# joaotavora/raytracing-one-weekend

Measured on AMD Instinct MI355X. Metric: Msamples/sec (W×H×spp) on cover scene; achieved HBM GB/s vs peak, higher is better.
Workload: dtype f64

## Files before the change

raytracing-one-weekend_amd/csrc/rtow_trace_body.h:

```cpp

#include <hip/hip_runtime.h>
#include <stdint.h>
#include <type_traits>

#include "rtow_device.h"

#ifndef RTOW_SUFFIX
#error "define RTOW_SUFFIX"
#endif
#define RTOW_CAT2(a, b) a##b
#define RTOW_CAT(a, b) RTOW_CAT2(a, b)

namespace rtow {
namespace {
#include "rtow_trace_math.h"
#include "rtow_trace_rng.h"
#include "rtow_trace_hit.h"
#include "rtow_trace_stamps.h"
#include "rtow_trace_bvh.h"
#include "rtow_trace_grid.h"
#include "rtow_trace_bvh4.h"
#ifndef RTOW_FAST_MATH
#include "rtow_trace_reftree.h"
#endif
#include "rtow_kernel_frame.h"

__device__ __forceinline__ uint32_t fastdiv(uint32_t n, FastDiv f) {
  const uint32_t t = __umulhi(n, f.magic);
  return f.shift == 255u ? n : (((n - t) >> 1) + t) >> f.shift;
}

constexpr uint32_t kItemBatch = 64;

__device__ __forceinline__ uint32_t lane_read(uint32_t src, uint32_t v) {
  return (uint32_t)__builtin_amdgcn_ds_bpermute((int)(src << 2), (int)v);
}
__device__ __forceinline__ double lane_read(uint32_t src, double v) {
  const unsigned long long b = (unsigned long long)__double_as_longlong(v);
  const uint32_t lo = lane_read(src, (uint32_t)b), hi = lane_read(src, (uint32_t)(b >> 32));
  return __longlong_as_double((long long)(((unsigned long long)hi << 32) | lo));
}
__device__ __forceinline__ double wave_bcast_f64(double v, int src_lane) {
  const unsigned long long b = (unsigned long long)__double_as_longlong(v);
  const uint32_t lo = (uint32_t)__builtin_amdgcn_readlane((int)(uint32_t)b, src_lane);
  const uint32_t hi = (uint32_t)__builtin_amdgcn_readlane((int)(uint32_t)(b >> 32), src_lane);
  return __longlong_as_double((long long)(((unsigned long long)hi << 32) | lo));
}

struct ItemPool {
  uint32_t next = 0, end = 0;
  unsigned long long seen = 0ull;
};

__device__ __forceinline__ FetchHead load_fetch_head(const RTOW_CONST FetchHead *p) {
  FetchHead h;
  h.n_items = p->n_items, h.n_items_first = p->n_items_first, h.empty_batch = p->empty_batch, h.W = p->W;
  h.partials = p->partials, h.counters = p->counters;
  return h;
}
__device__ __forceinline__ FetchDecode load_fetch_decode(const RTOW_CONST FetchDecode *p) {
  FetchDecode d;
  d.tile_w_log2 = p->tile_w_log2, d.tile_h_log2 = p->tile_h_log2, d.tile_table = p->tile_table;
  d.div_ns = FastDiv{p->div_ns.magic, p->div_ns.shift}, d.div_tpr = FastDiv{p->div_tpr.magic, p->div_tpr.shift};
  d.div_tpr_n = p->div_tpr_n, d.nstreams = p->nstreams, d.div_tile = FastDiv{p->div_tile.magic, p->div_tile.shift};
  d.rank = p->rank, d.nranks = p->nranks, d.tile_rows = p->tile_rows;
  d.sample_base = p->sample_base, d.spt = p->spt, d.spt_last = p->spt_last, d.npix_local = p->npix_local;
  return d;
}

__device__ __forceinline__ unsigned long long take_items(ItemPool &pool, unsigned long long need_mask, unsigned lane,
                                                         uint32_t n_waves, const FetchHead &kp) {
  const uint32_t want = (uint32_t)__popcll(need_mask);
  const uint32_t avail = pool.end - pool.next;
  const uint32_t rank = (uint32_t)__popcll(need_mask & ((1ull << lane) - 1ull));
  unsigned long long mine = (unsigned long long)pool.next + rank;
  if (want > avail) {
    const unsigned long long left =
        (unsigned long long)kp.n_items > pool.seen ? (unsigned long long)kp.n_items - pool.seen : 0ull;
#ifdef RTOW_NO_SHRINK
    uint32_t batch = kItemBatch;
    (void)left;
#else
    const bool sky = pool.seen >= (unsigned long long)kp.n_items_first;
    const uint32_t batch_max = sky ? kp.empty_batch : kItemBatch;
    uint32_t batch = (uint32_t)((sky ? left * (unsigned long long)(batch_max >> 6) : left) / ((unsigned long long)n_waves * 4ull));
    batch = batch > batch_max ? batch_max : batch;
    batch = batch < want - avail ? want - avail : batch;
#endif
    const int leader = __ffsll((long long)need_mask) - 1;
    unsigned long long base = pool.seen;
    if (pool.seen < (unsigned long long)kp.n_items) {
      if ((int)lane == leader) base = atomicAdd(&kp.counters[0], (unsigned long long)batch);
      base = __shfl(base, leader);
    }
    pool.seen = base + batch;
    if (rank >= avail) mine = base + (rank - avail);
    const unsigned long long nn = base + (want - avail), ne = base + batch;
    const unsigned long long cap = (unsigned long long)kp.n_items;
    pool.next = (uint32_t)(nn < cap ? nn : cap);
    pool.end = (uint32_t)(ne < cap ? ne : cap);
  } else {
    pool.next += want;
  }
  return mine;
}

struct ItemPos {
  uint32_t item, j, gi, sample0;
  int32_t count;
};
__device__ __forceinline__ ItemPos decode_item(const RTOW_CONST TraceParams *kp, const FetchHead &fh, uint32_t mine) {
  ItemPos ip;
  const FetchDecode kd = load_fetch_decode(kp);
  const uint32_t npix_local = kd.npix_local;
  const uint32_t qi = fh.n_items - 1u - mine;
  if (kd.tile_h_log2 == 0u) {
    const uint32_t k = fastdiv(qi, FastDiv{kp->div_npix.magic, kp->div_npix.shift});
    const uint32_t lp = qi - k * npix_local;
    const uint32_t lr = fastdiv(lp, FastDiv{kp->div_w.magic, kp->div_w.shift});
    ip.j = lp - lr * (uint32_t)fh.W;
    ip.item = k * npix_local + lp;
    const uint32_t q = fastdiv(lr, FastDiv{kd.div_tile.magic, kd.div_tile.shift});
    const uint32_t rr = lr - q * (uint32_t)kd.tile_rows;
    ip.gi = (q * (uint32_t)kd.nranks + (uint32_t)kd.rank) * (uint32_t)kd.tile_rows + rr;
    ip.sample0 = kd.sample_base + k * (uint32_t)kd.spt;
    ip.count = k + 1u == (uint32_t)kd.nstreams ? kd.spt_last : kd.spt;
    return ip;
  }
  const uint32_t g64 = qi >> 6, w = qi & 63u;
  const RTOW_CONST uint32_t *table = (const RTOW_CONST uint32_t *)kd.tile_table;
  ip.item = ip.j = ip.gi = ip.sample0 = 0u;
  ip.count = 0;
  for (;;) {
    const uint32_t ug = (uint32_t)__builtin_amdgcn_readfirstlane((int)g64);
    const uint32_t t = fastdiv(ug, FastDiv{kd.div_ns.magic, kd.div_ns.shift});
    const uint32_t k = ug - t * (uint32_t)kd.nstreams;
    const uint32_t tile = table[t];
    const uint32_t tr = fastdiv(tile, FastDiv{kd.div_tpr.magic, kd.div_tpr.shift});
    const uint32_t tc = tile - tr * kd.div_tpr_n;
    const uint32_t lr0 = tr << kd.tile_h_log2;
    const uint32_t q = fastdiv(lr0, FastDiv{kd.div_tile.magic, kd.div_tile.shift});
    const uint32_t gi0 = (q * (uint32_t)kd.nranks + (uint32_t)kd.rank) * (uint32_t)kd.tile_rows + (lr0 - q * (uint32_t)kd.tile_rows);
    const uint32_t item0 = k * npix_local + (tile << 6);
    const uint32_t j0 = tc << kd.tile_w_log2;
    const uint32_t s0 = kd.sample_base + k * (uint32_t)kd.spt;
    const int32_t cnt = k + 1u == (uint32_t)kd.nstreams ? kd.spt_last : kd.spt;
    if (g64 == ug) {
      ip.item = item0 + w;
      ip.j = j0 + (w & ((1u << kd.tile_w_log2) - 1u));
      ip.gi = gi0 + (w >> kd.tile_w_log2);
      ip.sample0 = s0;
      ip.count = cnt;
      break;
    }
  }
  return ip;
}

__device__ __forceinline__ void camera_ray(const TraceParams &P, Rng &g, uint32_t k0, uint32_t k1, uint32_t j,
                                           uint32_t gi, V3 &ro, V3 &rd, real &rtime) {
  g.r = 0u;
  const int from_top_i = P.H - (int)gi - 1;
  uint32_t o0, o1, o2, o3;
  philox4x32(g.r, g.sample, g.pixel, 0u, k0, k1, o0, o1, o2, o3);
  g.r += 1u;
  real ju, jv, jt, px, py;
  jitter_from_block(o0, o1, o2, ju, jv, jt);
  lens_from_block(o0, o1, o2, o3, px, py);
  const real u = fast_div((real)(int)j + ju, (real)(P.W - 1));
  const real v = fast_div((real)from_top_i + jv, (real)(P.H - 1));
#ifdef RTOW_REAL_F32
  const RTOW_CONST float *cm = (const RTOW_CONST float *)P.cam32;
#else
  cdptr cm = (cdptr)(const double *)P.cam;
#endif
  const real lens = cm[18], ct0 = cm[19], ct1 = cm[20];
  const real rdx = lens * px, rdy = lens * py;
  const V3 offset = V3{cm[3], cm[4], cm[5]} * rdx + V3{cm[6], cm[7], cm[8]} * rdy;
  const V3 from = V3{cm[0], cm[1], cm[2]} + offset;
  rd = V3{cm[15], cm[16], cm[17]} + u * V3{cm[9], cm[10], cm[11]} + v * V3{cm[12], cm[13], cm[14]} - from;
  ro = from;
  rtime = jt * (ct1 - ct0) + ct0;
}

__device__ __forceinline__ bool scatter_dir(Rng &g, uint32_t k0, uint32_t k1, int kind, real m_fuzz, real m_ir, V3 rd,
                                            V3 normal, bool front, V3 &dir) {
  uint32_t o0, o1, o2, o3;
  philox4x32(g.r, g.sample, g.pixel, 0u, k0, k1, o0, o1, o2, o3);
  g.r += 1u;
  V3 dirbase = {0, 0, 0};
  if (kind == 2) {
    const real ir = m_ir;
    const V3 unit = normalize(rd);
    const real cos_theta = dot(-unit, normal);
    const real sin_theta = fast_sqrt(real(1.0) - cos_theta * cos_theta);
    const real ratio = front ? fast_rcp(ir) : ir;
    bool refl = ratio * sin_theta > real(1.0);
    if (!refl) {
      real r0 = fast_div(real(1.0) - ratio, real(1.0) + ratio);
      r0 = r0 * r0;
      const real x = real(1.0) - cos_theta;
      const real x2 = x * x;
      const real R = r0 + (real(1.0) - r0) * (x2 * x2 * x);
      refl = R > coin_from_block(o0, o1, o3);
    }
    dirbase = refl ? reflect(unit, normal) : refract(unit, normal, ratio);
  } else if (kind == 1) {
    dirbase = reflect(rd, normal);
  }
  const V3 rnd = ball_from_block(o0, o1, o2, o3);
  bool absorbed = false;
  if (kind == 0) {
    absorbed = rabs(normal.x - rnd.x) < real(1e-8) && rabs(normal.y - rnd.y) < real(1e-8) &&
               rabs(normal.z - rnd.z) < real(1e-8);
    dir = normal + rnd;
  } else {
    dir = dirbase + m_fuzz * rnd;
  }
  return !absorbed;
}

template <int KERNEL, bool LDS, bool STAMPS = false, int SPEC = 0, bool COUNT = true>
__global__ void __launch_bounds__(KERNEL >= 2 && KERNEL <= 4 ? 1024 : 256)
    RTOW_CAT(rtow_trace_, RTOW_SUFFIX)(const TraceParams P) {
  const DevScene &sc = P.sc;
  const uint32_t k0 = P.seed_lo, k1 = P.seed_hi;
  const unsigned lane = lane_id();
  [[maybe_unused]] const uint32_t lane_g = blockIdx.x * blockDim.x + threadIdx.x;

  Image<LDS> im;
  [[maybe_unused]] Bvh4Reader<LDS> im4;
  stage_scene<KERNEL, LDS>(sc, im, im4);

  bool done = false;
  bool need_sample = true;
  bool pending_hit = false;
  int s_left = 0;
  uint32_t item = 0xffffffffu;
  uint32_t j = 0;
  uint32_t gi = 0;
  V3d acc = {0.0, 0.0, 0.0};
  V3 ro = {0, 0, 0}, rd = {0, 0, 1};
  real rtime = 0;
  int depth = 0;
  [[maybe_unused]] int nb = 0;
#ifdef RTOW_FAST_MATH
  V3 throughput = {1, 1, 1};
#endif
  Rng g = {0, 0, 0};
#ifdef RTOW_TAILSTAT
  constexpr bool kCount = true;
#else
  constexpr bool kCount = COUNT || STAMPS;
#endif
  WalkCount<kCount> nseg, nnode, nprim;
  [[maybe_unused]] float t_resume = 0.0f;
  [[maybe_unused]] uint32_t w_cur = 0x1fffffu, w_sa = 0u;
  Closest best;
  best.t = 0;
  best.prim = -1;
  bool helping = false;
  bool holding = false;
  uint32_t partners = 0u;
  int n_out = 0;
  uint32_t tail_left = P.tail_bound;
  asm volatile("" : "+v"(tail_left));
  ItemPool pool;
  const uint32_t n_waves = (gridDim.x * blockDim.x) >> 6;
#ifdef RTOW_TAILSTAT
  unsigned long long ts_start = __builtin_amdgcn_s_memrealtime(), ts_empty = 0ull;
  uint32_t ts_trips = 0u, ts_trips_after = 0u, ts_live = 0u, ts_left = 0u, ts_pool = 0u;
#endif
  Stamps<STAMPS> stamps;
  stamps.start();
  unsigned long long t_empty = 0ull;
  unsigned long long trips_after_empty = 0ull;
  if constexpr (STAMPS) {
    if (lane == 0) atomicMin(P.t_origin, (unsigned long long)__builtin_amdgcn_s_memrealtime());
  }

  for (;;) {
    bool need_item = false;
    if (!done && need_sample && s_left <= 0) {
      if (helping) {
        helping = false;
        holding = true;
        done = true;
      } else if (n_out == 0) {
        need_item = true;
      }
    }
    unsigned long long need_mask = __ballot(need_item);
    if (need_mask != 0ull && (uint32_t)__popcll(need_mask) < P.fetch_votes && __ballot(!done && !need_item) != 0ull) {
      need_mask = 0ull;
      need_item = false;
    }
    if (need_mask != 0ull) {
      const RTOW_CONST TraceParams *kp = (const RTOW_CONST TraceParams *)__builtin_amdgcn_kernarg_segment_ptr();
      asm volatile("" : "+s"(kp));
      const FetchHead fh = load_fetch_head(kp);
      if (need_item && item != 0xffffffffu) {
        double *dst = fh.partials + (size_t)item * 3;
        dst[0] = acc.x;
        dst[1] = acc.y;
        dst[2] = acc.z;
        item = 0xffffffffu;
      }
      const unsigned long long mine = take_items(pool, need_mask, lane, n_waves, fh);
      if (need_item) {
        if (mine >= (unsigned long long)fh.n_items) {
          done = true;
#ifdef RTOW_TAILSTAT
          if (ts_empty == 0ull) ts_empty = 1ull;
#endif
          if constexpr (STAMPS) {
            if (t_empty == 0ull) t_empty = __builtin_amdgcn_s_memrealtime();
          }
        } else {
          const ItemPos ip = decode_item(kp, fh, (uint32_t)mine);
          item = ip.item;
          j = ip.j;
          gi = ip.gi;
          g.pixel = gi * (uint32_t)fh.W + j;
          g.sample = ip.sample0;
          s_left = ip.count;
          acc = {0.0, 0.0, 0.0};
        }
      }
    }
#ifdef RTOW_TAILSTAT
    {
      const bool first = __ballot(ts_empty == 1ull) != 0ull && __ballot(ts_empty > 1ull) == 0ull;
      if (first) {
        const unsigned long long now = __builtin_amdgcn_s_memrealtime();
        ts_live = (uint32_t)__popcll(__ballot(!done));
        uint32_t sl = (!done && s_left > 0) ? (uint32_t)s_left : 0u;
        for (int off = 32; off >= 1; off >>= 1) sl += __shfl_xor(sl, off);
        ts_left = sl;
        ts_pool = pool.end - pool.next;
        ts_empty = now < 2ull ? 2ull : now;
      } else if (__ballot(ts_empty > 1ull) != 0ull) {
        ts_empty = (unsigned long long)__shfl((long long)ts_empty, __ffsll((long long)__ballot(ts_empty > 1ull)) - 1);
      }
      ++ts_trips;
      if (__ballot(ts_empty > 1ull) != 0ull) ++ts_trips_after;
    }
#endif
    if (__ballot(done) != 0ull) {
#ifdef RTOW_DONATE_R2
      const bool ready = !done && need_sample && s_left <= 0 && n_out > 0;
      if (__ballot(ready) != 0ull) {
        const uint32_t h = partners & 63u;
        const uint32_t src = ready ? h : lane;
        const uint32_t partner_holds = lane_read(src, (uint32_t)holding);
        const bool take = ready && partner_holds != 0u;
        const V3d c = {lane_read(src, acc.x), lane_read(src, acc.y), lane_read(src, acc.z)};
        const uint32_t ow = holding ? partners : lane;
        const bool o_take = lane_read(ow, (uint32_t)take) != 0u;
        const uint32_t o_h = lane_read(ow, h);
        if (take) {
          acc = acc + c;
          partners >>= 6;
          --n_out;
        }
        if (holding && o_take && o_h == lane) holding = false;
      }
      const bool can_give = !done && !helping && s_left >= 2 && n_out < 5;
#else
      unsigned long long rm = __ballot(!done && need_sample && s_left <= 0 && n_out > 0);
      while (rm != 0ull) {
        const int o = __ffsll((long long)rm) - 1;
        rm &= rm - 1ull;
        const uint32_t want_sample = (uint32_t)__builtin_amdgcn_readlane((int)g.sample, o);
        const uint32_t want_pixel = (uint32_t)__builtin_amdgcn_readlane((int)g.pixel, o);
        const unsigned long long held =
            __ballot(holding && partners == (uint32_t)o && g.sample == want_sample + 1u && g.pixel == want_pixel);
        if (held != 0ull) {
          const int h = __ffsll((long long)held) - 1;
          const V3d c = {wave_bcast_f64(acc.x, h), wave_bcast_f64(acc.y, h), wave_bcast_f64(acc.z, h)};
          if ((int)lane == o) {
            acc = acc + c;
            ++g.sample;
            --n_out;
          }
          if ((int)lane == h) holding = false;
          if (__builtin_amdgcn_readlane(n_out, o) > 0) rm |= 1ull << o;
        }
      }
      const bool can_give = !done && !helping && s_left >= 2;
#endif
      const bool can_help = done && !holding;
      const unsigned long long gm = __ballot(can_give), hm = __ballot(can_help);
      if (gm != 0ull && hm != 0ull) {
        const uint32_t ng = (uint32_t)__popcll(gm), nh = (uint32_t)__popcll(hm);
        const uint32_t cnt = ng < nh ? ng : nh;
        const uint32_t grank = lanes_below(gm), hrank = lanes_below(hm);
        const uint32_t giver_k = (uint32_t)__builtin_amdgcn_ds_permute(
            (int)((can_give ? grank : ng + (lane - grank)) << 2), (int)lane);
        const bool gives = can_give && grank < cnt;
        const bool helps = can_help && hrank < cnt;
        const uint32_t my_giver = lane_read(helps ? hrank : lane, giver_k);
#ifdef RTOW_DONATE_R2
        const uint32_t helper_k = (uint32_t)__builtin_amdgcn_ds_permute(
            (int)((can_help ? hrank : nh + (lane - hrank)) << 2), (int)lane);
        const uint32_t my_helper = lane_read(gives ? grank : lane, helper_k);
#endif
        const uint32_t gsrc = helps ? my_giver : lane;
        const uint32_t o_j = lane_read(gsrc, j), o_gi = lane_read(gsrc, gi);
        const uint32_t o_pixel = lane_read(gsrc, g.pixel), o_sample = lane_read(gsrc, g.sample);
        const uint32_t o_left = lane_read(gsrc, (uint32_t)s_left);
        if (gives) {
          s_left -= 1;
#ifdef RTOW_DONATE_R2
          partners = (partners << 6) | my_helper;
#endif
          ++n_out;
        }
        if (helps) {
          j = o_j;
          gi = o_gi;
          g.pixel = o_pixel;
          g.sample = o_sample + o_left - 1u;
          s_left = 1;
          need_sample = true;
          acc = {0.0, 0.0, 0.0};
          helping = true;
          done = false;
          partners = my_giver;
        }
      }
      if (tail_left == 0u) {
        if (!done || holding) {
          const RTOW_CONST TraceParams *kpt = (const RTOW_CONST TraceParams *)__builtin_amdgcn_kernarg_segment_ptr();
          atomicAdd(&P.counters[47], 1ull);
          atomicAdd(kpt->dropped, 1ull);
        }
        done = true;
        helping = false;
        holding = false;
        n_out = 0;
      } else {
        --tail_left;
      }
    }
    if (__ballot(!done || holding) == 0ull) break;
    stamps.mark(RG_FETCH);

    const bool live = !done && !(need_sample && s_left <= 0);

    const bool do_regen = live && need_sample;
    const bool do_scat = live && pending_hit;
    V3 normal = anyv3();
    bool front = true;
    int mi = 0, kind = 0;
    real m_fuzz = anyv(real(0)), m_ir = anyv(real(0));
#ifdef RTOW_FAST_MATH
    V3 m_att = anyv3();
#endif
    if (do_scat) {
      ro = ro + rd * best.t;
      const int pid = best.prim;
      if constexpr (KERNEL == 4) {
        const uint32_t r = sc.b4_off_tri + 96u * (uint32_t)pid;
        const vd2 q4 = im4.t2(r + 64u), q5 = im4.t2(r + 80u);
        normal = {(real)q4.y, (real)q5.x, (real)q5.y};
        mi = (int)im4.u32(sc.b4_off_pmat + 4u * (uint32_t)pid);
        const uint32_t mr = sc.b4_off_mats + 48u * (uint32_t)mi;
        const vd2 m1 = im4.d2(mr + 16u), m2 = im4.d2(mr + 32u);
#ifdef RTOW_FAST_MATH
        const vd2 m0 = im4.d2(mr);
        m_att = V3{(real)m0.x, (real)m0.y, (real)m1.x};
#endif
        m_fuzz = (real)m1.y;
        m_ir = (real)m2.x;
        kind = (int)(__double_as_longlong(m2.y) & 0xffffffffll);
      } else if constexpr (KERNEL >= 2 && KERNEL <= 4) {
        const uint32_t o_sph = KERNEL == 3 ? sc.g_off_sph : sc.off_sph;
        const uint32_t o_mov = KERNEL == 3 ? sc.g_off_mov : sc.off_mov;
        const uint32_t o_tri = KERNEL == 3 ? sc.g_off_tri : sc.off_tri;
        const uint32_t o_pmat = KERNEL == 3 ? sc.g_off_pmat : sc.off_pmat;
        const uint32_t o_mats = KERNEL == 3 ? sc.g_off_mats : sc.off_mats;
        if constexpr ((SPEC & 3) == 1) __builtin_assume(pid < sc.n_sph);
        if constexpr ((SPEC & 3) == 2) __builtin_assume(pid < sc.n_sph + sc.n_mov);
        if ((SPEC & 3) != 0 || pid < sc.n_sph + sc.n_mov) {
          V3 center;
          bool inward;
          if (pid < sc.n_sph) {
            const double2 p0 = im.d2(o_sph + 32u * (uint32_t)pid), p1 = im.d2(o_sph + 32u * (uint32_t)pid + 16u);
            center = {(real)p0.x, (real)p0.y, (real)p1.x};
            inward = p1.y < 0.0;
          } else {
            const uint32_t r = o_mov + 64u * (uint32_t)(pid - sc.n_sph);
            const double2 p0 = im.d2(r), p1 = im.d2(r + 16u), p2 = im.d2(r + 32u), p3 = im.d2(r + 48u);
#ifdef RTOW_REAL_F32
            center = {(real)p0.x + rtime * (real)p1.y, (real)p0.y + rtime * (real)p2.x, (real)p1.x + rtime * (real)p2.y};
#else
            center = {p0.x + rtime * p1.y, p0.y + rtime * p2.x, p1.x + rtime * p2.y};
#endif
            inward = p3.x < 0.0;
          }
          normal = normalize(ro - center);
          front = (dot(rd, normal) < real(0.0)) ^ inward;
          normal = front ? normal : -normal;
        } else {
#ifdef RTOW_REAL_F32
          const uint32_t r = o_tri + 48u * (uint32_t)(pid - sc.n_sph - sc.n_mov);
          const float4 q2 = im.f4(r + 32u);
          normal = {q2.y, q2.z, q2.w};
#else
          const uint32_t r = o_tri + 96u * (uint32_t)(pid - sc.n_sph - sc.n_mov);
          const double2 q4 = im.d2(r + 64u), q5 = im.d2(r + 80u);
          normal = {q4.y, q5.x, q5.y};
#endif
        }
        mi = (int)im.u32(o_pmat + 4u * (uint32_t)pid);
        const uint32_t mr = o_mats + 48u * (uint32_t)mi;
        const double2 m1 = im.d2(mr + 16u), m2 = im.d2(mr + 32u);
#ifdef RTOW_FAST_MATH
        const double2 m0 = im.d2(mr);
        m_att = V3{(real)m0.x, (real)m0.y, (real)m1.x};
#endif
        m_fuzz = (real)m1.y;
        m_ir = (real)m2.x;
        kind = (int)(__double_as_longlong(m2.y) & 0xffffffffll);
      } else {
        if (pid < sc.n_sph + sc.n_mov) {
          V3 center;
          bool inward;
          if (pid < sc.n_sph) {
            const double *q = sc.sph + 4 * (size_t)pid;
            center = {(real)q[0], (real)q[1], (real)q[2]};
            inward = sc.sph_r[pid] < 0.0;
          } else {
            const double *q = sc.mov + 8 * (size_t)(pid - sc.n_sph);
#ifdef RTOW_REAL_F32
            center = {(real)q[0] + rtime * (real)q[3], (real)q[1] + rtime * (real)q[4], (real)q[2] + rtime * (real)q[5]};
#else
            center = {q[0] + rtime * q[3], q[1] + rtime * q[4], q[2] + rtime * q[5]};
#endif
            inward = q[7] < 0.0;
          }
          normal = normalize(ro - center);
          front = (dot(rd, normal) < real(0.0)) ^ inward;
          normal = front ? normal : -normal;
        } else {
          const double *q = sc.tri + 12 * (size_t)(pid - sc.n_sph - sc.n_mov);
          normal = {(real)q[9], (real)q[10], (real)q[11]};
        }
        mi = sc.prim_mat[pid];
        const DevMaterial *m = sc.mats + mi;
#ifdef RTOW_FAST_MATH
        m_att = V3{(real)m->att[0], (real)m->att[1], (real)m->att[2]};
#endif
        kind = m->kind;
        m_fuzz = (real)m->fuzz;
        m_ir = (real)m->ir;
      }

    }
    stage_prio<kPrioRng>();
    uint32_t o0 = anyv(0u), o1 = anyv(0u), o2 = anyv(0u), o3 = anyv(0u);
    if (do_regen) g.r = 0u;
    if (do_regen || do_scat) {
      philox4x32(g.r, g.sample, g.pixel, 0u, k0, k1, o0, o1, o2, o3);
      g.r += 1u;
    }
    if constexpr (STAMPS) {
      if (__ballot(do_regen || do_scat) != 0ull) stamps.blocks += 1;
    }
    V3 dirbase = anyv3();
    real s_ang = anyv(real(0)), s_arg = anyv(real(0)), s_z = anyv(real(0));
    uint32_t s_b = anyv(0u);
    if (do_regen) {
      s_b = (o0 & 0x7ffu) | ((o1 & 0x7ffu) << 11) | ((o2 & 0x3ffu) << 22);
      s_ang = (real)(s_b & 0x3fffffffu) * real(0x1p-30 * kHalfPi);
      s_arg = (real)o3 * real(0x1p-32);
    }
    if (do_scat) {
      s_z = (real)(o0 >> 8) * real(0x1p-24);
      s_ang = (real)(o1 >> 8) * real(0x1p-24 * kHalfPi);
      s_arg = real(1.0) - s_z * s_z;
    }
    real s_sn = anyv(real(0)), s_cs = anyv(real(0)), s_sq = anyv(real(0));
    if (do_regen || do_scat) {
      opaque(s_ang);
      s_sn = sin_quarter(s_ang);
      s_cs = sin_quarter(real(kHalfPi) - s_ang);
      s_sq = fast_sqrt(s_arg);
    }
    if (do_scat) {
      if (kind == 2) {
        const real ir = m_ir;
        const V3 unit = normalize(rd);
        const real cos_theta = dot(-unit, normal);
        const real sin_theta = fast_sqrt(real(1.0) - cos_theta * cos_theta);
        const real ratio = front ? fast_rcp(ir) : ir;
        bool refl = ratio * sin_theta > real(1.0);
        if (!refl) {
          real r0 = fast_div(real(1.0) - ratio, real(1.0) + ratio);
          r0 = r0 * r0;
          const real x = real(1.0) - cos_theta;
          const real x2 = x * x;
          const real R = r0 + (real(1.0) - r0) * (x2 * x2 * x);
          refl = R > coin_from_block(o0, o1, o3);
        }
        dirbase = refl ? reflect(unit, normal) : refract(unit, normal, ratio);
      } else if (kind == 1) {
        dirbase = reflect(rd, normal);
      }
    }
    if (do_regen) {
      const int from_top_i = P.H - (int)gi - 1;
      real ju, jv, jt;
      jitter_from_block(o0, o1, o2, ju, jv, jt);
#ifdef RTOW_FAST_MATH
      const RTOW_CONST TraceParams *kq = (const RTOW_CONST TraceParams *)__builtin_amdgcn_kernarg_segment_ptr();
      asm volatile("" : "+s"(kq));
      const real u = ((real)(int)j + ju) * (real)kq->inv_wm1;
      const real v = ((real)from_top_i + jv) * (real)kq->inv_hm1;
#else
      const real u = fast_div((real)(int)j + ju, (real)(P.W - 1));
      const real v = fast_div((real)from_top_i + jv, (real)(P.H - 1));
#endif
#ifdef RTOW_REAL_F32
      const RTOW_CONST float *cm = (const RTOW_CONST float *)P.cam32;
#else
      cdptr cm = (cdptr)(const double *)P.cam;
#endif
      const real lens = cm[18], ct0 = cm[19], ct1 = cm[20];
      real px, py;
      {
        const uint32_t q = s_b >> 30;
        const real cx = (q & 1u) ? s_sn : s_cs, sy = (q & 1u) ? s_cs : s_sn;
        px = s_sq * ((q == 1u || q == 2u) ? -cx : cx);
        py = s_sq * (q >= 2u ? -sy : sy);
      }
      const real rdx = lens * px, rdy = lens * py;
      const V3 offset = V3{cm[3], cm[4], cm[5]} * rdx + V3{cm[6], cm[7], cm[8]} * rdy;
      const V3 from = V3{cm[0], cm[1], cm[2]} + offset;
      rd = V3{cm[15], cm[16], cm[17]} + u * V3{cm[9], cm[10], cm[11]} + v * V3{cm[12], cm[13], cm[14]} - from;
      ro = from;
      rtime = jt * (ct1 - ct0) + ct0;
      depth = P.max_child_rays;
      nb = 0;
#ifdef RTOW_FAST_MATH
      throughput = {1, 1, 1};
#endif
      need_sample = false;
    }
    if (do_scat) {
      pending_hit = false;
      bool absorbed = false;
      const real s_r = (real)max(max(o2 & 0xffffu, o2 >> 16), o3 & 0xffffu) * real(0x1p-16);
      const real s_rs = s_r * s_sq;
      const V3 rnd = V3{s_rs * s_cs, s_rs * s_sn, s_r * s_z};
      if (kind == 0) {
        absorbed = rabs(normal.x - rnd.x) < real(1e-8) && rabs(normal.y - rnd.y) < real(1e-8) &&
                   rabs(normal.z - rnd.z) < real(1e-8);
        rd = normal + rnd;
      } else {
        rd = dirbase + m_fuzz * rnd;
      }
      if (absorbed) {
        need_sample = true;
        --s_left;
        ++g.sample;
      } else {
#ifdef RTOW_FAST_MATH
        throughput = throughput * m_att;
#else
        P.stack[(size_t)nb * P.n_lanes + lane_g] = (uint32_t)mi;
#endif
        ++nb;
        --depth;
      }
    }
    stage_prio<kPrioStage>();
    const bool tracing = live && !need_sample;

    stamps.mark(RG_REGEN, __ballot(do_regen || do_scat));
    if constexpr (STAMPS) {
      stamps.trips += 1;
      if (t_empty != 0ull) trips_after_empty += 1;
      stamps.tail = t_empty != 0ull;
    }
    if constexpr (KERNEL != 3 && KERNEL != 4) {
      best.t = 0;
      best.prim = -1;
    }
    if constexpr (KERNEL == 4) {
      best = closest_hit_bvh4<LDS, STAMPS>(im4, sc, P, ro, rd, rtime, tracing, lane_g, nnode, nprim, stamps, best, w_cur, w_sa,
                                           P.walk_cap, P.walk_max_open);
    } else if constexpr (KERNEL == 3) {
      if constexpr (STAMPS) stamps.primary = __ballot(tracing && depth == P.max_child_rays);
      const RTOW_CONST TraceParams *kw = (const RTOW_CONST TraceParams *)__builtin_amdgcn_kernarg_segment_ptr();
      if constexpr ((SPEC & 3) != 0) asm volatile("" : "+s"(kw));
      best = closest_hit_grid<LDS, STAMPS, (SPEC & 3), (SPEC & (int)kSpecFlatY) != 0>(
          im, sc, ro, rd, rtime, tracing, nnode, nprim, stamps, best, t_resume, P.walk_cap, P.walk_max_open, P.leaf_votes,
          &kw->walk);
    } else if constexpr (KERNEL == 2) {
      best = closest_hit_bvh<LDS, STAMPS>(im, sc, ro, rd, rtime, tracing, nnode, nprim, stamps);
    } else if constexpr (KERNEL == 5) {
#ifndef RTOW_FAST_MATH
      if (tracing) best = closest_hit_reftree(sc, to_f64(ro), to_f64(rd), (double)rtime, nnode.n, nprim.n);
#endif
    } else {
      best = closest_hit_stream(sc, to_f64(ro), to_f64(rd), (double)rtime, tracing);
    }

    stamps.mark(RG_WALK, __ballot(tracing));
    bool arrived = tracing;
    if constexpr (KERNEL == 3) arrived = tracing && !(t_resume > 0.0f);
    if constexpr (KERNEL == 4) arrived = tracing && w_cur == 0x1fffffu;
    if (arrived) {
      ++nseg;
      if (best.prim >= 0) {
        if (depth <= 0)
          need_sample = true;
        else
          pending_hit = true;
      } else {
        const V3 unit = normalize(rd);
        const real t = real(0.5) * (unit.y + real(+1.0));
        V3 c = (real(1.0) - t) * V3{1, 1, 1} + t * V3{real(0.5), real(0.7), real(1.0)};
#ifdef RTOW_FAST_MATH
        c = throughput * c;
#else
        for (int q = nb - 1; q >= 0; --q) {
          const uint32_t smi = P.stack[(size_t)q * P.n_lanes + lane_g];
          if constexpr (KERNEL == 4) {
            const uint32_t mr = sc.b4_off_mats + 48u * smi;
            const vd2 a0 = im4.d2(mr), a1 = im4.d2(mr + 16u);
            c = V3{(real)a0.x, (real)a0.y, (real)a1.x} * c;
          } else if constexpr (KERNEL >= 2 && KERNEL <= 4) {
            const uint32_t mr = (KERNEL == 3 ? sc.g_off_mats : sc.off_mats) + 48u * smi;
            const double2 a0 = im.d2(mr), a1 = im.d2(mr + 16u);
            c = V3{(real)a0.x, (real)a0.y, (real)a1.x} * c;
          } else {
            const DevMaterial *m = sc.mats + smi;
            c = V3{(real)m->att[0], (real)m->att[1], (real)m->att[2]} * c;
          }
        }
#endif
        {
          V3d cd = to_f64(c);
          asm volatile("" : "+v"(cd.x), "+v"(cd.y), "+v"(cd.z));
          acc = acc + cd;
        }
        need_sample = true;
      }
      if (need_sample) {
        --s_left;
        ++g.sample;
      }
    }
    stamps.mark(RG_SHADE, __ballot(arrived));
  }
  if constexpr (STAMPS) {
    if (lane == 0)
    {
      const unsigned long long tend = __builtin_amdgcn_s_memrealtime();
      atomicAdd(&P.counters[4], tend - P.t_origin[0]);
      atomicMin(&P.counters[5], tend - P.t_origin[0]);
      atomicMax(&P.counters[6], tend - P.t_origin[0]);
      atomicAdd(&P.counters[7], t_empty - P.t_origin[0]);
      {
        const unsigned long long after = tend - t_empty;
        unsigned bin = (unsigned)(after / 20000ull);
        bin = bin > 5u ? 5u : bin;
        atomicAdd(&P.counters[17 + bin], 1ull);
        atomicMax(&P.counters[40], trips_after_empty);
        if (bin >= 2u) {
          atomicAdd(&P.counters[41], trips_after_empty);
          atomicAdd(&P.counters[42], after);
          atomicAdd(&P.counters[43], 1ull);
        }
      }
      for (int r = 0; r < RG_COUNT; ++r) atomicAdd(&P.counters[8 + r], stamps.t[r]);
      for (int r = 0; r < RG_COUNT; ++r) atomicAdd(&P.counters[29 + r], stamps.tt[r]);
      atomicAdd(&P.counters[37], trips_after_empty);
      atomicAdd(&P.counters[38], tend - t_empty);
      for (int r = 0; r < RG_COUNT; ++r) atomicAdd(&P.counters[23 + r], stamps.lt[r]);
      atomicAdd(&P.counters[34], stamps.step_lanes);
      atomicAdd(&P.counters[44], stamps.blocks);
      atomicAdd(&P.counters[36], stamps.block_lanes);
      atomicAdd(&P.counters[35], stamps.leaf_lanes);
      atomicAdd(&P.counters[45], stamps.iters_cam);
      atomicAdd(&P.counters[46], stamps.phases_cam);
      atomicAdd(&P.counters[13], stamps.iters);
      atomicAdd(&P.counters[14], stamps.trips);
      atomicAdd(&P.counters[15], stamps.phases);
    }
  }

#ifdef RTOW_TAILSTAT
  if (lane == 0 && P.spill != nullptr) {
    unsigned long long *ts = (unsigned long long *)P.spill + (size_t)((blockIdx.x * blockDim.x + threadIdx.x) >> 6) * 8;
    ts[0] = ts_start;
    ts[1] = ts_empty;
    ts[2] = __builtin_amdgcn_s_memrealtime();
    ts[3] = ts_trips;
    ts[4] = ts_trips_after;
    ts[5] = ts_live;
    ts[6] = ts_left;
    ts[7] = ts_pool;
  }
#endif
  if constexpr (kCount) {
    unsigned long long t0 = nseg.value(), t1 = nprim.value(), t2 = nnode.value();
#pragma unroll
    for (int off = 32; off >= 1; off >>= 1) {
      t0 += __shfl_down(t0, off);
      t1 += __shfl_down(t1, off);
      t2 += __shfl_down(t2, off);
    }
    if (lane == 0) {
      atomicAdd(&P.counters[1], t0);
      if (KERNEL >= 2) {
        atomicAdd(&P.counters[2], t1);
        atomicAdd(&P.counters[3], t2);
      }
    }
  }
}

#include "rtow_trace_sm4.h"

}

#include "rtow_kernel_launch.h"

template <int K, bool L, bool S, int SPEC = 0, bool COUNT = true>
static KernelVariant<TraceParams> trace_kernel(unsigned lds_bytes) {
  return kernel_variant<RTOW_CAT(rtow_trace_, RTOW_SUFFIX)<K, L, S, SPEC, COUNT>, TraceParams>(lds_bytes);
}
template <int K, bool L, int SPEC = 0>
static KernelVariant<TraceParams> trace_kernel_by_count(unsigned lds_bytes, bool count) {
#ifndef RTOW_REAL_F32
  if (!count) return trace_kernel<K, L, false, SPEC, false>(lds_bytes);
#endif
  return trace_kernel<K, L, false, SPEC, true>(lds_bytes);
}
template <bool L, bool S>
static KernelVariant<TraceParams> trace4_kernel(unsigned lds_bytes) {
  return kernel_variant<RTOW_CAT(rtow_trace4_, RTOW_SUFFIX)<L, S>, TraceParams>(lds_bytes);
}

static KernelVariant<TraceParams> trace_variant(int kernel, unsigned lds_bytes, uint32_t spec, bool b4_full,
                                                bool b4_trips, bool count = true, bool *counted = nullptr) {
  const bool lds = lds_bytes > 0;
  bool dummy;
  bool &cnt = counted ? *counted : dummy;
  cnt = true;
#ifndef RTOW_REAL_F32
  const bool has_nocount = (kernel == 3 && lds && (spec & 3u) != 0u) || (kernel == 4 && b4_trips);
  if (has_nocount) cnt = count;
#endif
  switch (kernel) {
    case 1: return trace_kernel<1, false, false>(lds_bytes);
    case 2: return lds ? trace_kernel<2, true, false>(lds_bytes) : trace_kernel<2, false, false>(0);
    case 3:
      if (lds && spec == kSpecStaticSpheres) return trace_kernel_by_count<3, true, 1>(lds_bytes, cnt);
      if (lds && spec == kSpecMovingSpheres) return trace_kernel_by_count<3, true, 2>(lds_bytes, cnt);
      if (lds && spec == (kSpecStaticSpheres | kSpecFlatY)) return trace_kernel_by_count<3, true, 1 | (int)kSpecFlatY>(lds_bytes, cnt);
      if (lds && spec == (kSpecMovingSpheres | kSpecFlatY)) return trace_kernel_by_count<3, true, 2 | (int)kSpecFlatY>(lds_bytes, cnt);
      cnt = true;
      return lds ? trace_kernel<3, true, false>(lds_bytes) : trace_kernel<3, false, false>(0);
    case 4:
      if (b4_trips) return b4_full ? trace_kernel_by_count<4, true>(lds_bytes, cnt) : trace_kernel_by_count<4, false>(lds_bytes, cnt);
      return b4_full ? trace4_kernel<true, false>(lds_bytes) : trace4_kernel<false, false>(lds_bytes);
    case 4 + 16:
      if (b4_trips) return b4_full ? trace_kernel<4, true, true>(lds_bytes) : trace_kernel<4, false, true>(lds_bytes);
      return b4_full ? trace4_kernel<true, true>(lds_bytes) : trace4_kernel<false, true>(lds_bytes);
#ifndef RTOW_FAST_MATH
    case 5: return trace_kernel<5, false, false>(0);
#endif
    case 2 + 16: return trace_kernel<2, true, true>(lds_bytes);
    case 3 + 16: return trace_kernel<3, true, true>(lds_bytes);
    default: return {};
  }
}

int RTOW_CAT(launch_trace_, RTOW_SUFFIX)(const TraceParams &p, int kernel, int grid, int block,
                                         unsigned lds_bytes, void *stream, bool count, bool *counted) {
  const KernelVariant<TraceParams> v =
      trace_variant(kernel, lds_bytes, p.spec, p.sc.b4_half == 0u, p.b4_trips != 0u, count, counted);
  return v.fn ? v.launch(p, grid, block, v.lds_bytes, (hipStream_t)stream) : (int)hipErrorInvalidValue;
}

int RTOW_CAT(trace_occupancy_, RTOW_SUFFIX)(int kernel, int block, unsigned lds_bytes) {
  const KernelVariant<TraceParams> v = trace_variant(kernel, lds_bytes, kSpecGeneric, true, true);
  return resident_blocks(v.fn, block, v.lds_bytes, nullptr);
}

}
```

raytracing-one-weekend_amd/csrc/rtow_trace_math.h:

```cpp
#pragma once

#define RTOW_CONST __attribute__((address_space(4)))
typedef const RTOW_CONST double *cdptr;

#ifdef RTOW_REAL_F32
typedef float real;
#else
typedef double real;
#endif

template <class T>
struct Vec3 {
  T x, y, z;
};
typedef Vec3<real> V3;
typedef Vec3<double> V3d;
template <class T>
__device__ __forceinline__ T anyv(T) {
  T x;
  asm volatile("" : "=v"(x));
  return x;
}
__device__ __forceinline__ V3 anyv3() { return V3{anyv(real(0)), anyv(real(0)), anyv(real(0))}; }
constexpr int kPrioRng = 0, kPrioSetup = 1, kPrioStage = 2, kPrioLeaf = 3;
template <int P>
__device__ __forceinline__ void stage_prio() {
#ifndef RTOW_NO_STAGE_PRIO
  __builtin_amdgcn_s_setprio(P);
#endif
}
template <class T>
__device__ __forceinline__ Vec3<T> operator+(Vec3<T> a, Vec3<T> b) { return {a.x + b.x, a.y + b.y, a.z + b.z}; }
template <class T>
__device__ __forceinline__ Vec3<T> operator-(Vec3<T> a, Vec3<T> b) { return {a.x - b.x, a.y - b.y, a.z - b.z}; }
template <class T>
__device__ __forceinline__ Vec3<T> operator-(Vec3<T> a) { return {-a.x, -a.y, -a.z}; }
template <class T>
__device__ __forceinline__ Vec3<T> operator*(Vec3<T> a, Vec3<T> b) { return {a.x * b.x, a.y * b.y, a.z * b.z}; }
template <class T>
__device__ __forceinline__ Vec3<T> operator*(Vec3<T> a, T s) { return {a.x * s, a.y * s, a.z * s}; }
template <class T>
__device__ __forceinline__ Vec3<T> operator*(T s, Vec3<T> a) { return {s * a.x, s * a.y, s * a.z}; }
template <class T>
__device__ __forceinline__ T dot(Vec3<T> a, Vec3<T> b) { return a.x * b.x + a.y * b.y + a.z * b.z; }
template <class T>
__device__ __forceinline__ Vec3<T> cross(Vec3<T> x, Vec3<T> y) {
  return {x.y * y.z - y.y * x.z, x.z * y.x - y.z * x.x, x.x * y.y - y.x * x.y};
}
__device__ __forceinline__ V3d to_f64(Vec3<float> v) { return {(double)v.x, (double)v.y, (double)v.z}; }
__device__ __forceinline__ V3d to_f64(V3d v) { return v; }
#ifdef RTOW_FAST_MATH
__device__ __forceinline__ double fast_rsqrt(double x) {
  const double y = __builtin_amdgcn_rsq(x);
#ifdef RTOW_SQRT_ORDER3
  const double z = (x * y) * y;
  return y * __builtin_fma(z, __builtin_fma(z, 0.375, -1.25), 1.875);
#else
  const double e = __builtin_fma(-(x * y), y, 1.0);
  return __builtin_fma(y * 0.5, e, y);
#endif
}
__device__ __forceinline__ double fast_sqrt_pos(double x) {
  const double y = __builtin_amdgcn_rsq(x);
#ifdef RTOW_SQRT_ORDER3
  const double s = x * y, z = s * y;
  return s * __builtin_fma(z, __builtin_fma(z, 0.375, -1.25), 1.875);
#else
  const double s = x * y, h = y * 0.5;
  const double e = __builtin_fma(-s, h, 0.5);
  return __builtin_fma(s, e, s);
#endif
}
__device__ __forceinline__ double fast_sqrt(double x) {
  if (!(x > 0.0)) return 0.0;
  return fast_sqrt_pos(x);
}
__device__ __forceinline__ double fast_rcp(double x) {
  const double y = __builtin_amdgcn_rcp(x);
  const double e = __builtin_fma(-x, y, 1.0);
  return __builtin_fma(y, __builtin_fma(e, e, e), y);
}
__device__ __forceinline__ double fast_div(double n, double d) { return n * fast_rcp(d); }
#else
__device__ __forceinline__ double fast_div(double n, double d) { return n / d; }
__device__ __forceinline__ double fast_sqrt(double x) { return sqrt(x); }
__device__ __forceinline__ double fast_sqrt_pos(double x) { return sqrt(x); }
__device__ __forceinline__ double fast_rcp(double x) { return 1.0 / x; }
__device__ __forceinline__ double fast_rsqrt(double x) { return 1.0 / sqrt(x); }
#endif
__device__ __forceinline__ float fast_rsqrt(float x) {
  float y = __builtin_amdgcn_rsqf(x);
  return y * (1.5f - 0.5f * x * y * y);
}
__device__ __forceinline__ float fast_sqrt(float x) { return x > 0.0f ? __builtin_amdgcn_sqrtf(x) : 0.0f; }
__device__ __forceinline__ float fast_sqrt_pos(float x) { return __builtin_amdgcn_sqrtf(x); }
__device__ __forceinline__ float fast_rcp(float x) {
  float y = __builtin_amdgcn_rcpf(x);
  return y * (2.0f - x * y);
}
__device__ __forceinline__ float fast_div(float n, float d) { return n * fast_rcp(d); }
template <class T>
__device__ __forceinline__ Vec3<T> normalize(Vec3<T> v) { return v * fast_rsqrt(dot(v, v)); }
template <class T>
__device__ __forceinline__ Vec3<T> reflect(Vec3<T> I, Vec3<T> N) { return I - N * dot(N, I) * T(2.0); }
template <class T>
__device__ __forceinline__ Vec3<T> refract(Vec3<T> I, Vec3<T> N, T eta) {
  T d = dot(N, I);
  T k = T(1.0) - eta * eta * (T(1.0) - d * d);
  if (k >= T(0.0)) return eta * I - (eta * d + fast_sqrt(k)) * N;
  return {T(0.0), T(0.0), T(0.0)};
}

extern __shared__ __align__(16) unsigned char rtow_lds[];
typedef float vf4 __attribute__((ext_vector_type(4)));
typedef uint32_t vu4 __attribute__((ext_vector_type(4)));
typedef double vd2 __attribute__((ext_vector_type(2)));
typedef _Float16 vh4 __attribute__((ext_vector_type(4)));
#define RTOW_AS_LDS __attribute__((address_space(3)))
#define RTOW_AS_GLB __attribute__((address_space(1)))
template <class T>
__device__ __forceinline__ T lds_read(uint32_t off) {
#ifdef RTOW_LDS_SYMBOL
  return *(const RTOW_AS_LDS T *)((const RTOW_AS_LDS unsigned char *)rtow_lds + off);
#else
  return *(const RTOW_AS_LDS T *)(uintptr_t)off;
#endif
}
template <class T>
__device__ __forceinline__ void lds_write(uint32_t off, T v) {
#ifdef RTOW_LDS_SYMBOL
  *(RTOW_AS_LDS T *)((RTOW_AS_LDS unsigned char *)rtow_lds + off) = v;
#else
  *(RTOW_AS_LDS T *)(uintptr_t)off = v;
#endif
}
template <class T>
__device__ __forceinline__ T glb_read(const unsigned char *base, uint32_t off) {
  return *(const RTOW_AS_GLB T *)((const RTOW_AS_GLB unsigned char *)base + off);
}
```

Baseline: 17320.

## Keep per-lane state flags as wave-uniform ballot masks in scalar registers

Replaces the per-lane boolean state (done, need_sample, pending_hit, helping, holding) with 64-bit lane masks built by ballot, so the state machine runs on scalar registers and scalar logic. Per-lane predicates are recovered with inverse_ballot only where divergent code needs them. The goal is fewer VGPRs and fewer per-iteration vector compares and ballots in the main persistent loop. In exchange the control flow is restructured, for example the absorbed and sky paths become separate mask-gated blocks, and the donate section converts back and forth between masks and bools, which adds conversion work and risks subtle behaviour changes.

```diff
diff --git a/raytracing-one-weekend_amd/csrc/rtow_trace_body.h b/raytracing-one-weekend_amd/csrc/rtow_trace_body.h
--- a/raytracing-one-weekend_amd/csrc/rtow_trace_body.h
+++ b/raytracing-one-weekend_amd/csrc/rtow_trace_body.h
@@ -232,9 +232,8 @@
   [[maybe_unused]] Bvh4Reader<LDS> im4;
   stage_scene<KERNEL, LDS>(sc, im, im4);
 
-  bool done = false;
-  bool need_sample = true;
-  bool pending_hit = false;
+  const lanemask m_all = vote(true);
+  lanemask m_done = 0ull, m_ns = m_all, m_ph = 0ull, m_help = 0ull, m_hold = 0ull;
   int s_left = 0;
   uint32_t item = 0xffffffffu;
   uint32_t j = 0;
@@ -259,8 +258,6 @@
   Closest best;
   best.t = 0;
   best.prim = -1;
-  bool helping = false;
-  bool holding = false;
   uint32_t partners = 0u;
   int n_out = 0;
   uint32_t tail_left = P.tail_bound;
@@ -280,26 +277,18 @@
   }
 
   for (;;) {
-    bool need_item = false;
-    if (!done && need_sample && s_left <= 0) {
-      if (helping) {
-        helping = false;
-        holding = true;
-        done = true;
-      } else if (n_out == 0) {
-        need_item = true;
-      }
-    }
-    unsigned long long need_mask = __ballot(need_item);
-    if (need_mask != 0ull && (uint32_t)__popcll(need_mask) < P.fetch_votes && __ballot(!done && !need_item) != 0ull) {
-      need_mask = 0ull;
-      need_item = false;
-    }
+    const lanemask m_end = m_ns & ~m_done & vote(s_left <= 0);
+    const lanemask m_handed = m_end & m_help;
+    m_help &= ~m_handed;
+    m_hold |= m_handed;
+    m_done |= m_handed;
+    lanemask need_mask = m_end & ~m_handed & vote(n_out == 0);
+    if (need_mask != 0ull && count_of(need_mask) < P.fetch_votes && (m_all & ~m_done & ~need_mask) != 0ull) need_mask = 0ull;
     if (need_mask != 0ull) {
       const RTOW_CONST TraceParams *kp = (const RTOW_CONST TraceParams *)__builtin_amdgcn_kernarg_segment_ptr();
       asm volatile("" : "+s"(kp));
       const FetchHead fh = load_fetch_head(kp);
-      if (need_item && item != 0xffffffffu) {
+      if (lanes_of(need_mask) && item != 0xffffffffu) {
         double *dst = fh.partials + (size_t)item * 3;
         dst[0] = acc.x;
         dst[1] = acc.y;
@@ -307,25 +296,25 @@
         item = 0xffffffffu;
       }
       const unsigned long long mine = take_items(pool, need_mask, lane, n_waves, fh);
-      if (need_item) {
-        if (mine >= (unsigned long long)fh.n_items) {
-          done = true;
+      const lanemask m_empty = need_mask & vote(mine >= (unsigned long long)fh.n_items);
+      m_done |= m_empty;
+      if (lanes_of(m_empty)) {
 #ifdef RTOW_TAILSTAT
-          if (ts_empty == 0ull) ts_empty = 1ull;
-#endif
-          if constexpr (STAMPS) {
-            if (t_empty == 0ull) t_empty = __builtin_amdgcn_s_memrealtime();
-          }
-        } else {
-          const ItemPos ip = decode_item(kp, fh, (uint32_t)mine);
-          item = ip.item;
-          j = ip.j;
-          gi = ip.gi;
-          g.pixel = gi * (uint32_t)fh.W + j;
-          g.sample = ip.sample0;
-          s_left = ip.count;
-          acc = {0.0, 0.0, 0.0};
-        }
+        if (ts_empty == 0ull) ts_empty = 1ull;
+#endif
+        if constexpr (STAMPS) {
+          if (t_empty == 0ull) t_empty = __builtin_amdgcn_s_memrealtime();
+        }
+      }
+      if (lanes_of(need_mask & ~m_empty)) {
+        const ItemPos ip = decode_item(kp, fh, (uint32_t)mine);
+        item = ip.item;
+        j = ip.j;
+        gi = ip.gi;
+        g.pixel = gi * (uint32_t)fh.W + j;
+        g.sample = ip.sample0;
+        s_left = ip.count;
+        acc = {0.0, 0.0, 0.0};
       }
     }
 #ifdef RTOW_TAILSTAT
@@ -333,8 +322,8 @@
       const bool first = __ballot(ts_empty == 1ull) != 0ull && __ballot(ts_empty > 1ull) == 0ull;
       if (first) {
         const unsigned long long now = __builtin_amdgcn_s_memrealtime();
-        ts_live = (uint32_t)__popcll(__ballot(!done));
-        uint32_t sl = (!done && s_left > 0) ? (uint32_t)s_left : 0u;
+        ts_live = count_of(m_all & ~m_done);
+        uint32_t sl = (lanes_of(m_all & ~m_done) && s_left > 0) ? (uint32_t)s_left : 0u;
         for (int off = 32; off >= 1; off >>= 1) sl += __shfl_xor(sl, off);
         ts_left = sl;
         ts_pool = pool.end - pool.next;
@@ -346,7 +335,8 @@
       if (__ballot(ts_empty > 1ull) != 0ull) ++ts_trips_after;
     }
 #endif
-    if (__ballot(done) != 0ull) {
+    if (m_done != 0ull) {
+      bool done = lanes_of(m_done), need_sample = lanes_of(m_ns), helping = lanes_of(m_help), holding = lanes_of(m_hold);
 #ifdef RTOW_DONATE_R2
       const bool ready = !done && need_sample && s_left <= 0 && n_out > 0;
       if (__ballot(ready) != 0ull) {
@@ -442,14 +432,15 @@
       } else {
         --tail_left;
       }
-    }
-    if (__ballot(!done || holding) == 0ull) break;
+      m_done = vote(done), m_ns = vote(need_sample), m_help = vote(helping), m_hold = vote(holding);
+    }
+    if (((m_all & ~m_done) | m_hold) == 0ull) break;
     stamps.mark(RG_FETCH);
 
-    const bool live = !done && !(need_sample && s_left <= 0);
-
-    const bool do_regen = live && need_sample;
-    const bool do_scat = live && pending_hit;
+    const lanemask m_live = m_all & ~m_done & ~(m_ns & vote(s_left <= 0));
+
+    const lanemask m_regen = m_live & m_ns, m_scat = m_live & m_ph;
+    const bool do_regen = lanes_of(m_regen), do_scat = lanes_of(m_scat);
     V3 normal = anyv3();
     bool front = true;
     int mi = 0, kind = 0;
@@ -566,7 +557,7 @@
       g.r += 1u;
     }
     if constexpr (STAMPS) {
-      if (__ballot(do_regen || do_scat) != 0ull) stamps.blocks += 1;
+      if ((m_regen | m_scat) != 0ull) stamps.blocks += 1;
     }
     V3 dirbase = anyv3();
     real s_ang = anyv(real(0)), s_arg = anyv(real(0)), s_z = anyv(real(0));
@@ -646,39 +637,42 @@
 #ifdef RTOW_FAST_MATH
       throughput = {1, 1, 1};
 #endif
-      need_sample = false;
-    }
+    }
+    m_ns &= ~m_regen;
+    m_ph &= ~m_scat;
+    V3 ab_d = anyv3();
     if (do_scat) {
-      pending_hit = false;
-      bool absorbed = false;
       const real s_r = (real)max(max(o2 & 0xffffu, o2 >> 16), o3 & 0xffffu) * real(0x1p-16);
       const real s_rs = s_r * s_sq;
       const V3 rnd = V3{s_rs * s_cs, s_rs * s_sn, s_r * s_z};
       if (kind == 0) {
-        absorbed = rabs(normal.x - rnd.x) < real(1e-8) && rabs(normal.y - rnd.y) < real(1e-8) &&
-                   rabs(normal.z - rnd.z) < real(1e-8);
+        ab_d = normal - rnd;
         rd = normal + rnd;
       } else {
         rd = dirbase + m_fuzz * rnd;
       }
-      if (absorbed) {
-        need_sample = true;
-        --s_left;
-        ++g.sample;
-      } else {
+    }
+    const lanemask m_absorbed = m_scat & vote(kind == 0) & vote(rabs(ab_d.x) < real(1e-8)) & vote(rabs(ab_d.y) < real(1e-8)) &
+                                vote(rabs(ab_d.z) < real(1e-8));
+    if (lanes_of(m_absorbed)) {
+      --s_left;
+      ++g.sample;
+    }
+    m_ns |= m_absorbed;
+    if (lanes_of(m_scat & ~m_absorbed)) {
 #ifdef RTOW_FAST_MATH
-        throughput = throughput * m_att;
-#else
-        P.stack[(size_t)nb * P.n_lanes + lane_g] = (uint32_t)mi;
-#endif
-        ++nb;
-        --depth;
-      }
+      throughput = throughput * m_att;
+#else
+      P.stack[(size_t)nb * P.n_lanes + lane_g] = (uint32_t)mi;
+#endif
+      ++nb;
+      --depth;
     }
     stage_prio<kPrioStage>();
-    const bool tracing = live && !need_sample;
-
-    stamps.mark(RG_REGEN, __ballot(do_regen || do_scat));
+    const lanemask m_tracing = m_live & ~m_ns;
+    [[maybe_unused]] const bool tracing = lanes_of(m_tracing);
+
+    stamps.mark(RG_REGEN, m_regen | m_scat);
     if constexpr (STAMPS) {
       stamps.trips += 1;
       if (t_empty != 0ull) trips_after_empty += 1;
@@ -688,16 +682,18 @@
       best.t = 0;
       best.prim = -1;
     }
+    [[maybe_unused]] lanemask m_open = 0ull;
     if constexpr (KERNEL == 4) {
       best = closest_hit_bvh4<LDS, STAMPS>(im4, sc, P, ro, rd, rtime, tracing, lane_g, nnode, nprim, stamps, best, w_cur, w_sa,
                                            P.walk_cap, P.walk_max_open);
     } else if constexpr (KERNEL == 3) {
-      if constexpr (STAMPS) stamps.primary = __ballot(tracing && depth == P.max_child_rays);
+      if constexpr (STAMPS) stamps.primary = m_tracing & vote(depth == P.max_child_rays);
       const RTOW_CONST TraceParams *kw = (const RTOW_CONST TraceParams *)__builtin_amdgcn_kernarg_segment_ptr();
       if constexpr ((SPEC & 3) != 0) asm volatile("" : "+s"(kw));
       best = closest_hit_grid<LDS, STAMPS, (SPEC & 3), (SPEC & (int)kSpecFlatY) != 0>(
-          im, sc, ro, rd, rtime, tracing, nnode, nprim, stamps, best, t_resume, P.walk_cap, P.walk_max_open, P.leaf_votes,
-          &kw->walk);
+          im, sc, ro, rd, rtime, tracing, nnode, nprim, stamps, best, t_resume, P.walk_cap, P.walk_max_open,
+          P.leaf_votes, &kw->walk);
+      m_open = vote(t_resume > 0.0f);
     } else if constexpr (KERNEL == 2) {
       best = closest_hit_bvh<LDS, STAMPS>(im, sc, ro, rd, rtime, tracing, nnode, nprim, stamps);
     } else if constexpr (KERNEL == 5) {
@@ -708,53 +704,51 @@
       best = closest_hit_stream(sc, to_f64(ro), to_f64(rd), (double)rtime, tracing);
     }
 
-    stamps.mark(RG_WALK, __ballot(tracing));
-    bool arrived = tracing;
-    if constexpr (KERNEL == 3) arrived = tracing && !(t_resume > 0.0f);
-    if constexpr (KERNEL == 4) arrived = tracing && w_cur == 0x1fffffu;
-    if (arrived) {
-      ++nseg;
-      if (best.prim >= 0) {
-        if (depth <= 0)
-          need_sample = true;
-        else
-          pending_hit = true;
-      } else {
-        const V3 unit = normalize(rd);
-        const real t = real(0.5) * (unit.y + real(+1.0));
-        V3 c = (real(1.0) - t) * V3{1, 1, 1} + t * V3{real(0.5), real(0.7), real(1.0)};
+    stamps.mark(RG_WALK, m_tracing);
+    lanemask m_arrived = m_tracing;
+    if constexpr (KERNEL == 3) m_arrived = m_tracing & ~m_open;
+    if constexpr (KERNEL == 4) m_arrived = m_tracing & vote(w_cur == 0x1fffffu);
+    const lanemask m_hit = m_arrived & vote(best.prim >= 0);
+    const lanemask m_black = m_hit & vote(depth <= 0);
+    const lanemask m_sky = m_arrived & ~m_hit;
+    m_ph |= m_hit & ~m_black;
+    if (lanes_of(m_arrived)) ++nseg;
+    if (lanes_of(m_sky)) {
+      const V3 unit = normalize(rd);
+      const real t = real(0.5) * (unit.y + real(+1.0));
+      V3 c = (real(1.0) - t) * V3{1, 1, 1} + t * V3{real(0.5), real(0.7), real(1.0)};
 #ifdef RTOW_FAST_MATH
-        c = throughput * c;
-#else
-        for (int q = nb - 1; q >= 0; --q) {
-          const uint32_t smi = P.stack[(size_t)q * P.n_lanes + lane_g];
-          if constexpr (KERNEL == 4) {
-            const uint32_t mr = sc.b4_off_mats + 48u * smi;
-            const vd2 a0 = im4.d2(mr), a1 = im4.d2(mr + 16u);
-            c = V3{(real)a0.x, (real)a0.y, (real)a1.x} * c;
-          } else if constexpr (KERNEL >= 2 && KERNEL <= 4) {
-            const uint32_t mr = (KERNEL == 3 ? sc.g_off_mats : sc.off_mats) + 48u * smi;
-            const double2 a0 = im.d2(mr), a1 = im.d2(mr + 16u);
-            c = V3{(real)a0.x, (real)a0.y, (real)a1.x} * c;
-          } else {
-            const DevMaterial *m = sc.mats + smi;
-            c = V3{(real)m->att[0], (real)m->att[1], (real)m->att[2]} * c;
-          }
-        }
-#endif
-        {
-          V3d cd = to_f64(c);
-          asm volatile("" : "+v"(cd.x), "+v"(cd.y), "+v"(cd.z));
-          acc = acc + cd;
-        }
-        need_sample = true;
-      }
-      if (need_sample) {
-        --s_left;
-        ++g.sample;
-      }
-    }
-    stamps.mark(RG_SHADE, __ballot(arrived));
+      c = throughput * c;
+#else
+      for (int q = nb - 1; q >= 0; --q) {
+        const uint32_t smi = P.stack[(size_t)q * P.n_lanes + lane_g];
+        if constexpr (KERNEL == 4) {
+          const uint32_t mr = sc.b4_off_mats + 48u * smi;
+          const vd2 a0 = im4.d2(mr), a1 = im4.d2(mr + 16u);
+          c = V3{(real)a0.x, (real)a0.y, (real)a1.x} * c;
+        } else if constexpr (KERNEL >= 2 && KERNEL <= 4) {
+          const uint32_t mr = (KERNEL == 3 ? sc.g_off_mats : sc.off_mats) + 48u * smi;
+          const double2 a0 = im.d2(mr), a1 = im.d2(mr + 16u);
+          c = V3{(real)a0.x, (real)a0.y, (real)a1.x} * c;
+        } else {
+          const DevMaterial *m = sc.mats + smi;
+          c = V3{(real)m->att[0], (real)m->att[1], (real)m->att[2]} * c;
+        }
+      }
+#endif
+      {
+        V3d cd = to_f64(c);
+        asm volatile("" : "+v"(cd.x), "+v"(cd.y), "+v"(cd.z));
+        acc = acc + cd;
+      }
+    }
+    const lanemask m_over = m_black | m_sky;
+    m_ns |= m_over;
+    if (lanes_of(m_over)) {
+      --s_left;
+      ++g.sample;
+    }
+    stamps.mark(RG_SHADE, m_arrived);
   }
   if constexpr (STAMPS) {
     if (lane == 0)
diff --git a/raytracing-one-weekend_amd/csrc/rtow_trace_math.h b/raytracing-one-weekend_amd/csrc/rtow_trace_math.h
--- a/raytracing-one-weekend_amd/csrc/rtow_trace_math.h
+++ b/raytracing-one-weekend_amd/csrc/rtow_trace_math.h
@@ -22,6 +22,10 @@
   return x;
 }
 __device__ __forceinline__ V3 anyv3() { return V3{anyv(real(0)), anyv(real(0)), anyv(real(0))}; }
+typedef unsigned long long lanemask;
+__device__ __forceinline__ lanemask vote(bool comparison) { return __builtin_amdgcn_ballot_w64(comparison); }
+__device__ __forceinline__ bool lanes_of(lanemask m) { return __builtin_amdgcn_inverse_ballot_w64(m); }
+__device__ __forceinline__ uint32_t count_of(lanemask m) { return (uint32_t)__popcll(m); }
 constexpr int kPrioRng = 0, kPrioSetup = 1, kPrioStage = 2, kPrioLeaf = 3;
 template <int P>
 __device__ __forceinline__ void stage_prio() {
```

Result: faster. 17670, median of 6 (+2.0%).
